# emdgroup/tnmf

Hardware: AMD Instinct MI355X
Metric: MU-iterations/sec (higher is better)
Workload: dtype f32

## Files before the change

### tnmf_amd/csrc/fft.h

```cpp
#pragma once
#include "common.h"

struct FftArgs {
    const void *src0, *src1, *src2;
    void *dst0, *dst1;
    long ps_src, ps_dst;
    int planes, rows, cols;
    int ld_src, ld_dst;
    int KX, KXP;
    int yoff, xoff;
    int N, M, C, Hy;
    int n0, ngroups, nper;
    int mgroups, mper;
    int clamp0;
    double reg;
};

enum FftOp {
    kFftRowsFwd = 0,
    kFftRowsInv,
    kFftRowsInv2,
    kFftRowsMu,
    kFftColsFwd,
    kFftColsInv,
    kFftContractR,
    kFftGradH,
    kFftGradW,
};

typedef int (*fft_run_fn)(int op, int dtype, const FftArgs *a, hipStream_t s);
#define TNMF_FFT_DECL(L) int fft_run_##L(int op, int dtype, const FftArgs *a, hipStream_t s)
TNMF_FFT_DECL(32);
TNMF_FFT_DECL(48);
TNMF_FFT_DECL(64);
TNMF_FFT_DECL(96);
TNMF_FFT_DECL(144);
TNMF_FFT_DECL(192);
TNMF_FFT_DECL(270);
TNMF_FFT_DECL(288);
TNMF_FFT_DECL(384);
TNMF_FFT_DECL(540);
TNMF_FFT_DECL(576);
#undef TNMF_FFT_DECL

bool mixed_has_reconstruct(const Geo &g, int dtype);
bool mixed_has_grad_W(const Geo &g, int dtype);
int mixed_reconstruct(const Geo &g, const void *Tsp, const void *WT, void *OT, int KX, int KXP, hipStream_t s);
int mixed_grad_W(const Geo &g, const void *Tsp, const void *VT, const void *RT, void *Gn, void *Gp, int KX, int KXP,
                 int ngroups, int nper, hipStream_t s);

#ifndef TNMF_MIX_W3_WAVES
#define TNMF_MIX_W3_WAVES 3
#endif
constexpr int kMixW3Atoms = 16, kMixW3Waves = TNMF_MIX_W3_WAVES, kMixW3MaxAy = 12;
constexpr long kMixW3MinBytes = 24L << 20;
constexpr int mix_w3_waves(int Ay) {
    const int w = Ay >= 8 ? 3 : (Ay >= 4 ? 4 : (Ay >= 2 ? 5 : 7));
    return kMixW3Waves < 3 ? kMixW3Waves : w;
}
bool mixed_grad_W3_takes(const Geo &g, int KXP);

int spectral_contract_R(const Geo &g, int dtype, const void *SH, const void *SW, void *SR, int Ly, int KX, int KXP,
                        hipStream_t s);
int spectral_grad_W(const Geo &g, int dtype, const void *SH, const void *SV, const void *SR, void *Gn, void *Gp, int Ly,
                    int KX, int KXP, int ngroups, int nper, hipStream_t s);

bool fft_has(const Geo &g, int dtype);
void fft_invalidate(tnmf_hip_ctx *ctx);
void fft_invalidate_H(tnmf_hip_ctx *ctx, const Geo &g, int dtype, const void *H);
void fft_bind(tnmf_hip_ctx *ctx, const Geo &g, int dtype, const void *H, const void *V);
void fft_unbind(tnmf_hip_ctx *ctx);
void fft_invalidate_W(tnmf_hip_ctx *ctx);
void fft_release(tnmf_hip_ctx *ctx);
int fft_reserve(tnmf_hip_ctx *ctx, const Geo &g, int dtype, bool with_window);

int fft_reconstruct(tnmf_hip_ctx *ctx, const Geo &g, int dtype, const void *W, const void *H, void *R, bool nonneg,
                    hipStream_t s);
int fft_grad_H(tnmf_hip_ctx *ctx, const Geo &g, int dtype, const void *V, const void *R, const void *W, void *neg,
               void *pos, hipStream_t s);
int fft_update_H(tnmf_hip_ctx *ctx, const Geo &g, int dtype, const void *V, const void *R, const void *W, void *H,
                 double reg, hipStream_t s);
int fft_grad_W(tnmf_hip_ctx *ctx, const Geo &g, int dtype, const void *V, const void *R, const void *H, void *neg,
               void *pos, bool nonneg, hipStream_t s);
```

### tnmf_amd/csrc/fft_mixed.hip

```cpp
#include "fft.h"

namespace {

typedef float f2v __attribute__((ext_vector_type(2)));
template <typename T>
struct cplx_of;
template <>
struct cplx_of<float> {
    using type = f2v;
};
template <typename T>
using cplx = typename cplx_of<T>::type;

__device__ __forceinline__ void cfma(f2v &acc, f2v a, f2v b) {
    asm("v_pk_fma_f32 %0, %1, %2, %0 op_sel:[0,0,0] op_sel_hi:[0,1,1]" : "+v"(acc) : "v"(a), "v"(b));
    asm("v_pk_fma_f32 %0, %1, %2, %0 op_sel:[1,1,0] op_sel_hi:[1,0,1] neg_lo:[0,1,0]" : "+v"(acc) : "v"(a), "v"(b));
}
__device__ __forceinline__ void cfmac(f2v &acc, f2v a, f2v b) {
    asm("v_pk_fma_f32 %0, %1, %2, %0 op_sel:[0,0,0] op_sel_hi:[0,1,1] neg_hi:[0,1,0]" : "+v"(acc) : "v"(a), "v"(b));
    asm("v_pk_fma_f32 %0, %1, %2, %0 op_sel:[1,1,0] op_sel_hi:[1,0,1]" : "+v"(acc) : "v"(a), "v"(b));
}
__device__ __forceinline__ void pfma_lo(f2v &acc, f2v x, f2v b) {
    asm("v_pk_fma_f32 %0, %1, %2, %0 op_sel:[0,0,0] op_sel_hi:[1,0,1]" : "+v"(acc) : "v"(x), "v"(b));
}
__device__ __forceinline__ void pfma_hi(f2v &acc, f2v x, f2v b) {
    asm("v_pk_fma_f32 %0, %1, %2, %0 op_sel:[0,1,0] op_sel_hi:[1,1,1]" : "+v"(acc) : "v"(x), "v"(b));
}

#define CHECK(rc_expr)                  \
    do {                                \
        const int _rc = (rc_expr);      \
        if (_rc != TNMF_OK) return _rc; \
    } while (0)

constexpr int kMixCols = 16;

template <typename T, int AY, int CG, int S, int STRIPS>
__global__ __launch_bounds__(kMixCols *STRIPS, 2) void k_mix_reconstruct(const cplx<T> *Tsp, const cplx<T> *WT,
                                                                      cplx<T> *OT, int M, int C, int Hy, int Dy, int KX,
                                                                      int KXP) {
    const int col = threadIdx.x & (kMixCols - 1), strip = threadIdx.x / kMixCols;
    const int kx = blockIdx.x * kMixCols + col, kxc = min(kx, KX - 1);
    const int y0 = (blockIdx.y * STRIPS + strip) * S, n = blockIdx.z;
    cplx<T> acc[CG][S];
#pragma unroll
    for (int c = 0; c < CG; ++c)
#pragma unroll
        for (int y = 0; y < S; ++y) acc[c][y] = {0, 0};
    static_assert(sizeof(cplx<T>) == 8, "float spectra");
    typedef unsigned u32x2v __attribute__((ext_vector_type(2)));
    auto ld = [](const __amdgpu_buffer_rsrc_t &rs, int lane_off, int row_off) {
        const u32x2v w2 = __builtin_amdgcn_raw_buffer_load_b64(rs, lane_off, row_off, 0);
        const unsigned re = w2[0], im = w2[1];
        return cplx<T>{__builtin_bit_cast(float, re), __builtin_bit_cast(float, im)};
    };
    const int rowb = KXP * 8;
    const long tplane = (long)Hy * KXP, wplane = (long)AY * KXP;
    const int lane_t = (y0 * KXP + kxc) * 8, lane_w = kxc * 8;
    const __amdgpu_buffer_rsrc_t wrs =
        __builtin_amdgcn_make_buffer_rsrc((void *)WT, 0, (int)((long)M * C * wplane * 8), 0x00020000);
    auto plane = [&](int m) {
        return __builtin_amdgcn_make_buffer_rsrc((void *)(Tsp + ((long)n * M + m) * tplane), 0, (int)(tplane * 8),
                                                 0x00020000);
    };
    cplx<T> t[S + AY - 1], tn[S + AY - 1];
    {
        const __amdgpu_buffer_rsrc_t rs = plane(0);
#pragma unroll
        for (int r = 0; r < S + AY - 1; ++r) t[r] = ld(rs, lane_t, r * rowb);
    }
    if constexpr (CG == 1) {
        constexpr int MC = 8, NT = kMixCols * STRIPS, ROWS = MC * AY, PIECES = ROWS * (kMixCols / 2);
        constexpr int NPP = (PIECES + NT - 1) / NT;
        typedef float f4v __attribute__((ext_vector_type(4)));
        __shared__ __align__(16) cplx<T> wl[2][ROWS * kMixCols];
        const cplx<T> *wsrc = WT + blockIdx.x * kMixCols;
        const int wrows = M * AY;
        f4v pre[NPP];
        auto wfetch = [&](int chunk) {
#pragma unroll
            for (int k = 0; k < NPP; ++k) {
                const int p = threadIdx.x + k * NT, row = min(chunk * ROWS + (p >> 3), wrows - 1);
                pre[k] = *reinterpret_cast<const f4v *>(wsrc + (long)row * KXP + 2 * (p & 7));
            }
        };
        auto wpark = [&](int buf) {
#pragma unroll
            for (int k = 0; k < NPP; ++k) {
                const int p = threadIdx.x + k * NT;
                if (p < PIECES) *reinterpret_cast<f4v *>(&wl[buf][(p >> 3) * kMixCols + 2 * (p & 7)]) = pre[k];
            }
        };
        wfetch(0);
        wpark(0);
        __syncthreads();
#pragma unroll 1
        for (int m0 = 0, ch = 0; m0 < M; m0 += MC, ++ch) {
            const int buf = ch & 1;
            const bool more = m0 + MC < M;
            if (more) wfetch(ch + 1);
#pragma unroll 1
            for (int mi = 0; mi < MC; ++mi) {
                const int m = m0 + mi;
                if (m >= M) break;
                cplx<T> w[AY];
#pragma unroll
                for (int a = 0; a < AY; ++a) w[a] = wl[buf][(mi * AY + (AY - 1 - a)) * kMixCols + col];
                {
                    const __amdgpu_buffer_rsrc_t rs = plane(min(m + 1, M - 1));
#pragma unroll
                    for (int r = 0; r < S + AY - 1; ++r) tn[r] = ld(rs, lane_t, r * rowb);
                }
#pragma unroll
                for (int a = 0; a < AY; ++a)
#pragma unroll
                    for (int y = 0; y < S; ++y) cfma(acc[0][y], t[y + a], w[a]);
#pragma unroll
                for (int r = 0; r < S + AY - 1; ++r) t[r] = tn[r];
            }
            if (more) wpark(buf ^ 1);
            __syncthreads();
        }
    } else {
#pragma unroll 1
    for (int m = 0; m < M; ++m) {
        cplx<T> w[CG][AY];
#pragma unroll
        for (int c = 0; c < CG; ++c) {
            const int wbase = ((m * C + min(c, C - 1)) * AY) * rowb;
#pragma unroll
            for (int a = 0; a < AY; ++a) w[c][a] = ld(wrs, lane_w, wbase + (AY - 1 - a) * rowb);
        }
        {
            const __amdgpu_buffer_rsrc_t rs = plane(min(m + 1, M - 1));
#pragma unroll
            for (int r = 0; r < S + AY - 1; ++r) tn[r] = ld(rs, lane_t, r * rowb);
        }
#pragma unroll
        for (int c = 0; c < CG; ++c)
#pragma unroll
            for (int a = 0; a < AY; ++a)
#pragma unroll
                for (int y = 0; y < S; ++y) cfma(acc[c][y], t[y + a], w[c][a]);
#pragma unroll
        for (int r = 0; r < S + AY - 1; ++r) t[r] = tn[r];
    }
    }
    if (kx >= KX) return;
#pragma unroll
    for (int c = 0; c < CG; ++c) {
        if (c >= C) break;
#pragma unroll
        for (int y = 0; y < S; ++y)
            if (y0 + y < Dy) OT[((long)n * C + c) * ((long)Dy * KXP) + (long)(y0 + y) * KXP + kx] = acc[c][y];
    }
}

template <typename T, int CG, int SAMPLES>
__global__ __launch_bounds__(kMixCols *SAMPLES) void k_mix_reconstruct_1d(const cplx<T> *Tsp, const cplx<T> *WT,
                                                                        cplx<T> *OT, int N, int M, int C, int KX,
                                                                        int KXP) {
    const int col = threadIdx.x & (kMixCols - 1), sub = threadIdx.x / kMixCols;
    const int kx = blockIdx.x * kMixCols + col, kxc = min(kx, KX - 1);
    const int n = blockIdx.y * SAMPLES + sub, nc = min(n, N - 1);
    cplx<T> acc[CG];
#pragma unroll
    for (int c = 0; c < CG; ++c) acc[c] = {0, 0};
    const cplx<T> *tp = Tsp + (long)nc * M * KXP + kxc;
    int m = 0;
    for (; m + 4 <= M; m += 4) {
        cplx<T> t[4];
#pragma unroll
        for (int q = 0; q < 4; ++q) t[q] = tp[(long)(m + q) * KXP];
#pragma unroll
        for (int q = 0; q < 4; ++q)
#pragma unroll
            for (int c = 0; c < CG; ++c) cfma(acc[c], t[q], WT[((long)(m + q) * C + min(c, C - 1)) * KXP + kxc]);
    }
    for (; m < M; ++m) {
        const cplx<T> t = tp[(long)m * KXP];
#pragma unroll
        for (int c = 0; c < CG; ++c) cfma(acc[c], t, WT[((long)m * C + min(c, C - 1)) * KXP + kxc]);
    }
    if (kx >= KX || n >= N) return;
#pragma unroll
    for (int c = 0; c < CG; ++c) {
        if (c >= C) break;
        OT[((long)n * C + c) * KXP + kx] = acc[c];
    }
}

template <typename T, int AY>
int launch_mix_reconstruct(const void *Tsp, const void *WT, void *OT, const Geo &g, int KX, int KXP, hipStream_t s) {
    const unsigned tiles = (unsigned)cdiv(KX, kMixCols);
    if constexpr (AY == 1) {
        if (g.Dy == 1) {
            constexpr int SAMPLES = 16;
            hipLaunchKernelGGL((k_mix_reconstruct_1d<T, 3, SAMPLES>), dim3(tiles, (unsigned)cdiv(g.N, SAMPLES)),
                               dim3(kMixCols * SAMPLES), 0, s, (const cplx<T> *)Tsp, (const cplx<T> *)WT, (cplx<T> *)OT,
                               g.N, g.M, g.C, KX, KXP);
            TNMF_LAUNCH_CHECK();
            return TNMF_OK;
        }
    }
    if (g.C == 1) {
        constexpr int S = 16, STRIPS = 8;
        hipLaunchKernelGGL((k_mix_reconstruct<T, AY, 1, S, STRIPS>),
                           dim3(tiles, (unsigned)cdiv(g.Dy, S * STRIPS), (unsigned)g.N), dim3(kMixCols * STRIPS), 0, s,
                           (const cplx<T> *)Tsp, (const cplx<T> *)WT, (cplx<T> *)OT, g.M, g.C, g.Hy, g.Dy, KX, KXP);
    } else {
        constexpr int S = 8, STRIPS = 8;
        hipLaunchKernelGGL((k_mix_reconstruct<T, AY, 3, S, STRIPS>),
                           dim3(tiles, (unsigned)cdiv(g.Dy, S * STRIPS), (unsigned)g.N), dim3(kMixCols * STRIPS), 0, s,
                           (const cplx<T> *)Tsp, (const cplx<T> *)WT, (cplx<T> *)OT, g.M, g.C, g.Hy, g.Dy, KX, KXP);
    }
    TNMF_LAUNCH_CHECK();
    return TNMF_OK;
}

template <typename T, int AY, int CG, int GROUPS>
__global__ __launch_bounds__(kMixCols *GROUPS, 2) void k_mix_grad_W(const cplx<T> *Tsp, const cplx<T> *VT,
                                                                 const cplx<T> *RT, cplx<T> *Gn, cplx<T> *Gp, int N,
                                                                 int M, int C, int Hy, int Dy, int KX, int KXP,
                                                                 int nper) {
    const int col = threadIdx.x & (kMixCols - 1), sub = threadIdx.x / kMixCols;
    const int kx = blockIdx.y * kMixCols + col, kxc = min(kx, KX - 1);
    const int m = blockIdx.x, grp = blockIdx.z * GROUPS + sub;
    cplx<T> an[CG][AY], ap[CG][AY];
#pragma unroll
    for (int c = 0; c < CG; ++c)
#pragma unroll
        for (int a = 0; a < AY; ++a) {
            an[c][a] = {0, 0};
            ap[c][a] = {0, 0};
        }
    const int nbeg = grp * nper, nend = min(N, nbeg + nper);
    const long tplane = (long)Hy * KXP, vplane = (long)Dy * KXP;
    static_assert(CG == 1, "one channel per thread");
#pragma unroll 1
    for (int n = nbeg; n < nend; ++n) {
        const cplx<T> *tp = Tsp + ((long)n * M + m) * tplane;
        const cplx<T> *vp = VT + (long)n * C * vplane, *rp = RT + (long)n * C * vplane;
        cplx<T> t[2 * AY - 1], v[AY], r[AY], tn[AY], vn[AY], rn[AY];
#pragma unroll
        for (int i = 0; i < 2 * AY - 1; ++i) t[i] = tp[(unsigned)(min(i, Hy - 1) * KXP + kxc)];
#pragma unroll
        for (int j = 0; j < AY; ++j) {
            const unsigned o = (unsigned)(min(j, Dy - 1) * KXP + kxc);
            v[j] = vp[o];
            r[j] = rp[o];
        }
#pragma unroll 1
        for (int yb = 0; yb < Dy; yb += AY) {
#pragma unroll
            for (int i = 0; i < AY; ++i) tn[i] = tp[(unsigned)(min(yb + 2 * AY - 1 + i, Hy - 1) * KXP + kxc)];
#pragma unroll
            for (int j = 0; j < AY; ++j) {
                const unsigned o = (unsigned)(min(yb + AY + j, Dy - 1) * KXP + kxc);
                vn[j] = vp[o];
                rn[j] = rp[o];
            }
#pragma unroll
            for (int j = 0; j < AY; ++j) {
                if (yb + j >= Dy) {
                    v[j] = {0, 0};
                    r[j] = {0, 0};
                }
#pragma unroll
                for (int a = 0; a < AY; ++a) {
                    cfmac(an[0][a], t[j + a], v[j]);
                    cfmac(ap[0][a], t[j + a], r[j]);
                }
            }
#pragma unroll
            for (int i = 0; i < AY - 1; ++i) t[i] = t[i + AY];
#pragma unroll
            for (int i = 0; i < AY; ++i) t[AY - 1 + i] = tn[i];
#pragma unroll
            for (int j = 0; j < AY; ++j) {
                v[j] = vn[j];
                r[j] = rn[j];
            }
        }
    }
    if (kx >= KX) return;
    const long gplane = (long)AY * KXP, gsize = (long)M * C * gplane;
#pragma unroll
    for (int c = 0; c < CG; ++c) {
        if (c >= C) break;
#pragma unroll
        for (int a = 0; a < AY; ++a) {
            const long o = (long)grp * gsize + ((long)m * C + c) * gplane + (long)a * KXP + kx;
            Gn[o] = an[c][a];
            Gp[o] = ap[c][a];
        }
    }
}

template <typename T, int AY, int GROUPS>
__global__ __launch_bounds__(kMixCols *GROUPS, 2) void k_mix_grad_W2(const cplx<T> *Tsp, const cplx<T> *VT,
                                                                  const cplx<T> *RT, cplx<T> *Gn, cplx<T> *Gp, int N,
                                                                  int M, int Hy, int Dy, int KX, int KXP, int nper,
                                                                  int gx, int gy, int gz) {
    constexpr int MA = 2, VS = 8, RS = (AY + 4 + VS - 1) / VS * VS, P = VS - 1;
    const int col = threadIdx.x & (kMixCols - 1), sub = threadIdx.x / kMixCols;
    int lin = blockIdx.x;
    {
        const int total = gx * gy * gz, whole = total / 8 * 8;
        if (lin < whole) lin = (lin & 7) * (whole / 8) + (lin >> 3);
    }
    const int bx = lin % gx, by = (lin / gx) % gy, bz = lin / (gx * gy);
    const int kx = by * kMixCols + col, kxc = min(kx, KX - 1);
    const int m0 = bx * MA, grp = bz * GROUPS + sub;
    const int m1 = min(m0 + 1, M - 1);
    cplx<T> an[MA][AY], ap[MA][AY];
#pragma unroll
    for (int q = 0; q < MA; ++q)
#pragma unroll
        for (int a = 0; a < AY; ++a) {
            an[q][a] = {0, 0};
            ap[q][a] = {0, 0};
        }
    static_assert(sizeof(cplx<T>) == 8, "float spectra");
    typedef unsigned u32x2v __attribute__((ext_vector_type(2)));
    const long tplane = (long)Hy * KXP, vplane = (long)Dy * KXP;
    const int nbeg0 = bz * GROUPS * nper, nbeg = nbeg0 + sub * nper;
    const int lane_t = (int)(((long)sub * nper * M * tplane + kxc) * 8);
    const int lane_v = (int)(((long)sub * nper * vplane + kxc) * 8);
    const int rowb = KXP * 8;
    auto ld = [](const __amdgpu_buffer_rsrc_t &rs, int lane_off, int row_off) {
        const u32x2v w = __builtin_amdgcn_raw_buffer_load_b64(rs, lane_off, row_off, 0);
        const unsigned re = w[0], im = w[1];
        return cplx<T>{__builtin_bit_cast(float, re), __builtin_bit_cast(float, im)};
    };
#pragma unroll 1
    for (int nr = 0; nr < nper; ++nr) {
        if (nbeg0 + nr >= N) break;
        if (nbeg + nr >= N) continue;
        const cplx<T> *tb = Tsp + ((long)(nbeg0 + nr) * M + m0) * tplane;
        const __amdgpu_buffer_rsrc_t t0 = __builtin_amdgcn_make_buffer_rsrc((void *)tb, 0, 0x7fffffff, 0x00020000);
        const __amdgpu_buffer_rsrc_t t1 =
            __builtin_amdgcn_make_buffer_rsrc((void *)(tb + (long)(m1 - m0) * tplane), 0, 0x7fffffff, 0x00020000);
        const __amdgpu_buffer_rsrc_t vb =
            __builtin_amdgcn_make_buffer_rsrc((void *)(VT + (long)(nbeg0 + nr) * vplane), 0, 0x7fffffff, 0x00020000);
        const __amdgpu_buffer_rsrc_t rb =
            __builtin_amdgcn_make_buffer_rsrc((void *)(RT + (long)(nbeg0 + nr) * vplane), 0, 0x7fffffff, 0x00020000);
        cplx<T> t[MA][RS], v[VS], r[VS];
#pragma unroll
        for (int i = 0; i < RS - 1; ++i) {
            const int o = min(i, Hy - 1) * rowb;
            t[0][i] = ld(t0, lane_t, o);
            t[1][i] = ld(t1, lane_t, o);
        }
#pragma unroll
        for (int i = 0; i < P; ++i) {
            const int o = min(i, Dy - 1) * rowb;
            v[i] = ld(vb, lane_v, o);
            r[i] = ld(rb, lane_v, o);
        }
#pragma unroll 1
        for (int yb = 0; yb < Dy; yb += RS) {
#pragma unroll
            for (int i = 0; i < RS; ++i) {
                const int y = yb + i;
                if (y >= Dy) break;
                {
                    const int o = min(y + RS - 1, Hy - 1) * rowb;
                    t[0][(i + RS - 1) % RS] = ld(t0, lane_t, o);
                    t[1][(i + RS - 1) % RS] = ld(t1, lane_t, o);
                    const int ov = min(y + P, Dy - 1) * rowb;
                    v[(i + P) % VS] = ld(vb, lane_v, ov);
                    r[(i + P) % VS] = ld(rb, lane_v, ov);
                }
                const cplx<T> vy = v[i % VS], ry = r[i % VS];
#pragma unroll
                for (int a = 0; a < AY; ++a) {
                    cfmac(an[0][a], t[0][(i + a) % RS], vy);
                    cfmac(ap[0][a], t[0][(i + a) % RS], ry);
                    cfmac(an[1][a], t[1][(i + a) % RS], vy);
                    cfmac(ap[1][a], t[1][(i + a) % RS], ry);
                }
            }
        }
    }
    if (kx >= KX) return;
    const long gplane = (long)AY * KXP, gsize = (long)M * gplane;
#pragma unroll
    for (int q = 0; q < MA; ++q) {
        if (m0 + q >= M) break;
#pragma unroll
        for (int a = 0; a < AY; ++a) {
            const long o = (long)grp * gsize + (long)(m0 + q) * gplane + (long)a * KXP + kx;
            Gn[o] = an[q][a];
            Gp[o] = ap[q][a];
        }
    }
}

#if defined(__HIP_DEVICE_COMPILE__)
#define TNMF_MIX_NO_DS_PAIRING __attribute__((target("no-load-store-opt")))
#else
#define TNMF_MIX_NO_DS_PAIRING
#endif
template <typename T, int AY>
__global__ __launch_bounds__(kMixCols *kMixW3Atoms, kMixW3Waves) TNMF_MIX_NO_DS_PAIRING void k_mix_grad_W3(
    const cplx<T> *Tsp, const cplx<T> *VT, const cplx<T> *RT, cplx<T> *Gn, cplx<T> *Gp, int N, int M, int Hy, int Dy,
    int KX, int KXP, int nper, int gx, int gy, int gz) {
    constexpr int NA = kMixW3Atoms, RS = 16, CH = RS, NT = kMixCols * NA;
    static_assert(AY + 4 <= RS && sizeof(cplx<T>) == 8 && NT == 2 * CH * (kMixCols / 2), "ring depth, float spectra");
    const int col = threadIdx.x & (kMixCols - 1), slot = threadIdx.x / kMixCols;
    int lin = blockIdx.x;
    {
        const int total = gx * gy * gz, whole = total / 8 * 8;
        if (lin < whole) lin = (lin & 7) * (whole / 8) + (lin >> 3);
    }
    const int bx = lin % gx, by = (lin / gx) % gy, grp = lin / (gx * gy);
    const int kx = by * kMixCols + col, kxc = min(kx, KX - 1);
    const int m = bx * NA + slot, mc = min(m, M - 1);
    f2v a1[AY], a2[AY], a3[AY];
#pragma unroll
    for (int a = 0; a < AY; ++a) a1[a] = a2[a] = a3[a] = {0, 0};
    typedef unsigned u32x2v __attribute__((ext_vector_type(2)));
    typedef float f4v __attribute__((ext_vector_type(4)));
    const long tplane = (long)Hy * KXP, vplane = (long)Dy * KXP;
    const int nbeg = grp * nper, nend = min(N, nbeg + nper);
    const int lane_t = (int)(((long)(mc - bx * NA) * tplane + kxc) * 8);
    const int rowb = KXP * 8;
    auto ld = [](const __amdgpu_buffer_rsrc_t &rs, int lane_off, int row_off) {
        const u32x2v w = __builtin_amdgcn_raw_buffer_load_b64(rs, lane_off, row_off, 0);
        const unsigned re = w[0], im = w[1];
        return cplx<T>{__builtin_bit_cast(float, re), __builtin_bit_cast(float, im)};
    };
    __shared__ __align__(16) f2v xl[2][3][CH * kMixCols];
    const int prow = threadIdx.x / kMixCols, ppair = (threadIdx.x >> 1) & (kMixCols / 2 - 1), pstream = threadIdx.x & 1;
    const cplx<T> *xsrc = (pstream ? RT : VT) + by * kMixCols + 2 * ppair;
    f4v pre;
    auto xfetch = [&](int n, int chunk) {
        pre = *reinterpret_cast<const f4v *>(xsrc + (long)n * vplane + (long)min(chunk * CH + prow, Dy - 1) * KXP);
    };
    auto xpark = [&](int buf) {
        auto swap1 = [](float v) {
            return __builtin_bit_cast(float,
                                      __builtin_amdgcn_update_dpp(0, __builtin_bit_cast(int, v), 0xB1, 0xf, 0xf, false));
        };
        const float oc = swap1(pstream ? pre[0] : pre[2]), od = swap1(pstream ? pre[1] : pre[3]);
        const float cv = pstream ? oc : pre[0], dv = pstream ? od : pre[1];
        const float cr = pstream ? pre[2] : oc, dr = pstream ? pre[3] : od;
        const int e = prow * kMixCols + 2 * ppair + pstream;
        xl[buf][0][e] = f2v{cv, cr};
        xl[buf][1][e] = f2v{cv + dv, cr + dr};
        xl[buf][2][e] = f2v{cv - dv, cr - dr};
    };
    xfetch(min(nbeg, N - 1), 0);
    xpark(0);
    __syncthreads();
    int buf = 0;
#pragma unroll 1
    for (int n = nbeg; n < nend; ++n) {
        const __amdgpu_buffer_rsrc_t t0 = __builtin_amdgcn_make_buffer_rsrc(
            (void *)(Tsp + ((long)n * M + bx * NA) * tplane), 0, 0x7fffffff, 0x00020000);
        cplx<T> t[RS];
        f2v sp[RS / 2];
#pragma unroll
        for (int i = 0; i < RS - 1; ++i) t[i] = ld(t0, lane_t, min(i, Hy - 1) * rowb);
#pragma unroll
        for (int i = 0; i < AY - 1; ++i) sp[i / 2][i & 1] = t[i][0] + t[i][1];
#pragma unroll 1
        for (int yb = 0; yb < Dy; yb += CH) {
            {
                const bool last = yb + CH >= Dy;
                xfetch(last ? min(n + 1, nend - 1) : n, last ? 0 : yb / CH + 1);
            }
            const f2v *x1 = &xl[buf][0][col], *x2 = &xl[buf][1][col], *x3 = &xl[buf][2][col];
#pragma unroll
            for (int i = 0; i < RS; ++i) {
                const int y = yb + i;
                if (y >= Dy) break;
                t[(i + RS - 1) % RS] = ld(t0, lane_t, min(y + RS - 1, Hy - 1) * rowb);
                {
                    const int j = (i + AY - 1) % RS;
                    sp[j / 2][j & 1] = t[j][0] + t[j][1];
                }
                const f2v c = x1[i * kMixCols], cpd = x2[i * kMixCols], cmd = x3[i * kMixCols];
#pragma unroll
                for (int a = 0; a < AY; ++a) {
                    const int j = (i + a) % RS;
                    if (j & 1)
                        pfma_hi(a1[a], c, sp[j / 2]);
                    else
                        pfma_lo(a1[a], c, sp[j / 2]);
                    pfma_lo(a2[a], cpd, t[j]);
                    pfma_hi(a3[a], cmd, t[j]);
                }
            }
            xpark(buf ^ 1);
            __syncthreads();
            buf ^= 1;
        }
    }
    if (kx >= KX || m >= M) return;
    const long gplane = (long)AY * KXP, gsize = (long)M * gplane;
#pragma unroll
    for (int a = 0; a < AY; ++a) {
        const long o = (long)grp * gsize + (long)m * gplane + (long)a * KXP + kx;
        Gn[o] = cplx<T>{a1[a][0] - a3[a][0], a1[a][0] - a2[a][0]};
        Gp[o] = cplx<T>{a1[a][1] - a3[a][1], a1[a][1] - a2[a][1]};
    }
}

template <typename T, int CG, int GROUPS>
__global__ __launch_bounds__(kMixCols *GROUPS) void k_mix_grad_W_1d(const cplx<T> *Tsp, const cplx<T> *VT, const cplx<T> *RT,
                                                                  cplx<T> *Gn, cplx<T> *Gp, int N, int M, int C, int KX,
                                                                  int KXP, int nper) {
    const int col = threadIdx.x & (kMixCols - 1), sub = threadIdx.x / kMixCols;
    const int kx = blockIdx.y * kMixCols + col, kxc = min(kx, KX - 1);
    const int m = blockIdx.x, grp = blockIdx.z * GROUPS + sub;
    cplx<T> an[CG], ap[CG];
#pragma unroll
    for (int c = 0; c < CG; ++c) {
        an[c] = {0, 0};
        ap[c] = {0, 0};
    }
    const int nbeg = grp * nper, nend = min(N, nbeg + nper);
    for (int n = nbeg; n < nend; ++n) {
        const cplx<T> t = Tsp[((long)n * M + m) * KXP + kxc];
#pragma unroll
        for (int c = 0; c < CG; ++c) {
            const long o = ((long)n * C + min(c, C - 1)) * KXP + kxc;
            cfmac(an[c], t, VT[o]);
            cfmac(ap[c], t, RT[o]);
        }
    }
    if (kx >= KX) return;
    const long gsize = (long)M * C * KXP;
#pragma unroll
    for (int c = 0; c < CG; ++c) {
        if (c >= C) break;
        const long o = (long)grp * gsize + ((long)m * C + c) * KXP + kx;
        Gn[o] = an[c];
        Gp[o] = ap[c];
    }
}

template <typename T, int AY>
int launch_mix_grad_W(const void *Tsp, const void *VT, const void *RT, void *Gn, void *Gp, const Geo &g, int KX,
                      int KXP, int ngroups, int nper, hipStream_t s) {
    constexpr int GROUPS = 4;
    if constexpr (AY == 1) {
        if (g.Dy == 1) {
            const dim3 grid((unsigned)g.M, (unsigned)cdiv(KX, kMixCols), (unsigned)cdiv(ngroups, GROUPS));
            hipLaunchKernelGGL((k_mix_grad_W_1d<T, 4, GROUPS>), grid, dim3(kMixCols * GROUPS), 0, s, (const cplx<T> *)Tsp,
                               (const cplx<T> *)VT, (const cplx<T> *)RT, (cplx<T> *)Gn, (cplx<T> *)Gp, g.N, g.M, g.C, KX,
                               KXP, nper);
            TNMF_LAUNCH_CHECK();
            return TNMF_OK;
        }
    }
    if constexpr (AY <= kMixW3MaxAy) {
        if (mixed_grad_W3_takes(g, KXP)) {
            const int gx = cdiv(g.M, kMixW3Atoms), gy = cdiv(KX, kMixCols), gz = ngroups;
            hipLaunchKernelGGL((k_mix_grad_W3<T, AY>), dim3((unsigned)(gx * gy * gz)), dim3(kMixCols * kMixW3Atoms),
                               kMixW3Waves == 2 ? 48u << 10 : 0u, s,
                               (const cplx<T> *)Tsp, (const cplx<T> *)VT, (const cplx<T> *)RT, (cplx<T> *)Gn,
                               (cplx<T> *)Gp, g.N, g.M, g.Hy, g.Dy, KX, KXP, nper, gx, gy, gz);
            TNMF_LAUNCH_CHECK();
            return TNMF_OK;
        }
    }
    if constexpr (AY <= 12) {
        const long span = ((long)(GROUPS - 1) * nper * g.M + 2) * g.Hy * KXP * 8;
        if (g.C == 1 && span < (1L << 31)) {
            const int gx = cdiv(g.M, 2), gy = cdiv(KX, kMixCols), gz = cdiv(ngroups, GROUPS);
            hipLaunchKernelGGL((k_mix_grad_W2<T, AY, GROUPS>), dim3((unsigned)(gx * gy * gz)), dim3(kMixCols * GROUPS), 0, s,
                               (const cplx<T> *)Tsp, (const cplx<T> *)VT, (const cplx<T> *)RT, (cplx<T> *)Gn,
                               (cplx<T> *)Gp, g.N, g.M, g.Hy, g.Dy, KX, KXP, nper, gx, gy, gz);
            TNMF_LAUNCH_CHECK();
            return TNMF_OK;
        }
    }
    const dim3 grid((unsigned)g.M, (unsigned)cdiv(KX, kMixCols), (unsigned)cdiv(ngroups, GROUPS));
    hipLaunchKernelGGL((k_mix_grad_W<T, AY, 1, GROUPS>), grid, dim3(kMixCols * GROUPS), 0, s, (const cplx<T> *)Tsp,
                       (const cplx<T> *)VT, (const cplx<T> *)RT, (cplx<T> *)Gn, (cplx<T> *)Gp, g.N, g.M, g.C, g.Hy, g.Dy,
                       KX, KXP, nper);
    TNMF_LAUNCH_CHECK();
    return TNMF_OK;
}

#define MIX_SWITCH(FN, ...)                                   \
    switch (g.Ay) {                                           \
        case 1: return FN<float, 1>(__VA_ARGS__);             \
        case 2: return FN<float, 2>(__VA_ARGS__);             \
        case 3: return FN<float, 3>(__VA_ARGS__);             \
        case 4: return FN<float, 4>(__VA_ARGS__);             \
        case 5: return FN<float, 5>(__VA_ARGS__);             \
        case 6: return FN<float, 6>(__VA_ARGS__);             \
        case 7: return FN<float, 7>(__VA_ARGS__);             \
        case 8: return FN<float, 8>(__VA_ARGS__);             \
        case 9: return FN<float, 9>(__VA_ARGS__);             \
        case 10: return FN<float, 10>(__VA_ARGS__);           \
        case 11: return FN<float, 11>(__VA_ARGS__);           \
        case 12: return FN<float, 12>(__VA_ARGS__);           \
        case 13: return FN<float, 13>(__VA_ARGS__);           \
        case 14: return FN<float, 14>(__VA_ARGS__);           \
        case 15: return FN<float, 15>(__VA_ARGS__);           \
        case 16: return FN<float, 16>(__VA_ARGS__);           \
        default: return TNMF_E_UNSUPPORTED;                   \
    }

}

bool mixed_has_reconstruct(const Geo &g, int dtype) {
    return dtype == 0 && g.Ay <= 16 && (g.C == 1 || (g.Dy == 1 && g.Ay == 1 && g.C <= 3));
}
bool mixed_has_grad_W(const Geo &g, int dtype) {
    return dtype == 0 && g.Ay <= 16 && (g.C == 1 || (g.Dy == 1 && g.Ay == 1 && g.C <= 4));
}

bool mixed_grad_W3_takes(const Geo &g, int KXP) {
#ifdef TNMF_MIX_NO_W3
    return false;
#endif
    const long span = (long)kMixW3Atoms * g.Hy * KXP * 8;
    const long spectra = (long)g.N * g.M * g.Hy * KXP * 8;
    return g.C == 1 && g.Ay <= kMixW3MaxAy && !(g.Dy == 1 && g.Ay == 1) && span < (1L << 31) && spectra >= kMixW3MinBytes;
}

int mixed_reconstruct(const Geo &g, const void *Tsp, const void *WT, void *OT, int KX, int KXP, hipStream_t s) {
    MIX_SWITCH(launch_mix_reconstruct, Tsp, WT, OT, g, KX, KXP, s);
}

int mixed_grad_W(const Geo &g, const void *Tsp, const void *VT, const void *RT, void *Gn, void *Gp, int KX, int KXP,
                 int ngroups, int nper, hipStream_t s) {
    MIX_SWITCH(launch_mix_grad_W, Tsp, VT, RT, Gn, Gp, g, KX, KXP, ngroups, nper, s);
}
```

Measured before the change: 217.0.

## Add LDS-staged mixed reconstruct kernel with buffer-load prefetch for large spectra

Adds a new reconstruct kernel that stages each atom's spectral rows and W taps into shared memory, using 128-bit buffer loads prefetched one atom ahead. Strips then read overlapping rows from LDS instead of re-reading global memory. It is chosen for C==1, Ay<=12 and spectra of at least 24 MiB. Dynamic shared memory is padded so that about three workgroups fit per CU. The cost is an extra barrier per atom and higher LDS use, which may limit occupancy.

```diff
diff --git a/tnmf_amd/csrc/fft.h b/tnmf_amd/csrc/fft.h
--- a/tnmf_amd/csrc/fft.h
+++ b/tnmf_amd/csrc/fft.h
@@ -60,6 +60,31 @@
 }
 bool mixed_grad_W3_takes(const Geo &g, int KXP);
 
+#ifndef TNMF_MIX_RSH_STRIPS
+#define TNMF_MIX_RSH_STRIPS 16
+#endif
+#ifndef TNMF_MIX_RSH_TILES
+#define TNMF_MIX_RSH_TILES 1
+#endif
+#ifndef TNMF_MIX_RSH_PER_CU
+#define TNMF_MIX_RSH_PER_CU 3
+#endif
+#ifndef TNMF_MIX_RSH_FENCE
+#define TNMF_MIX_RSH_FENCE 0
+#endif
+#ifndef TNMF_MIX_RSH_AUX
+#define TNMF_MIX_RSH_AUX 2
+#endif
+constexpr int kMixRShStrips = TNMF_MIX_RSH_STRIPS, kMixRShTiles = TNMF_MIX_RSH_TILES, kMixRShPerCU = TNMF_MIX_RSH_PER_CU;
+constexpr int kMixRShFence = TNMF_MIX_RSH_FENCE, kMixRShAux = TNMF_MIX_RSH_AUX;
+constexpr int kMixRShWaves = kMixRShPerCU * kMixRShStrips / 16, kMixRShMaxAy = 12;
+constexpr long kMixRShMinBytes = 24L << 20;
+constexpr unsigned mix_rsh_lds_bytes(int Ay) {
+    return kMixRShTiles * (((16 * kMixRShStrips + Ay - 1) * 17 + 1) / 2 * 2 + Ay * 16) * 8u;
+}
+constexpr int mix_rsh_waves(int Ay) { return kMixRShWaves; }
+bool mixed_reconstruct_sh_takes(const Geo &g, int KXP);
+
 int spectral_contract_R(const Geo &g, int dtype, const void *SH, const void *SW, void *SR, int Ly, int KX, int KXP,
                         hipStream_t s);
 int spectral_grad_W(const Geo &g, int dtype, const void *SH, const void *SV, const void *SR, void *Gn, void *Gp, int Ly,
diff --git a/tnmf_amd/csrc/fft_mixed.hip b/tnmf_amd/csrc/fft_mixed.hip
--- a/tnmf_amd/csrc/fft_mixed.hip
+++ b/tnmf_amd/csrc/fft_mixed.hip
@@ -156,6 +156,92 @@
     }
 }
 
+#if defined(__HIP_DEVICE_COMPILE__)
+#define TNMF_MIX_NO_DS_PAIRING __attribute__((target("no-load-store-opt")))
+#else
+#define TNMF_MIX_NO_DS_PAIRING
+#endif
+
+template <typename T, int AY, int STRIPS, int TILES>
+__global__ __launch_bounds__(kMixCols *STRIPS, kMixRShWaves) TNMF_MIX_NO_DS_PAIRING void k_mix_reconstruct_sh(
+    const cplx<T> *Tsp, const cplx<T> *WT, cplx<T> *OT, int M, int Hy, int Dy, int KX, int KXP) {
+    constexpr int S = 16, NT = kMixCols * STRIPS, ROWS = S * STRIPS + AY - 1, PITCH = kMixCols + 1;
+    constexpr int SEG = kMixCols / 2;
+    constexpr int PIECES = ROWS * SEG, NPP = (PIECES + NT - 1) / NT, WPIECES = AY * SEG;
+    constexpr int TROWS = (ROWS * PITCH + 1) / 2 * 2, TILE = TROWS + AY * kMixCols;
+    static_assert(sizeof(cplx<T>) == 8 && WPIECES <= NT && (TILES == 1 || TILES == 2), "float spectra, one W piece per thread");
+    static_assert(STRIPS != kMixRShStrips || TILES != kMixRShTiles || TILES * TILE * 8 == mix_rsh_lds_bytes(AY), "fft.h");
+    typedef unsigned u32x4v __attribute__((ext_vector_type(4)));
+    typedef float f4v __attribute__((ext_vector_type(4)));
+    __shared__ __align__(16) cplx<T> tile[TILES][TILE];
+    const int col = threadIdx.x & (kMixCols - 1), strip = threadIdx.x / kMixCols;
+    const int kx = blockIdx.x * kMixCols + col, colc = min(kx, KX - 1) - blockIdx.x * kMixCols;
+    const int yb = blockIdx.y * (S * STRIPS), y0 = yb + strip * S, n = blockIdx.z;
+    cplx<T> acc[S];
+#pragma unroll
+    for (int y = 0; y < S; ++y) acc[y] = {0, 0};
+    const long tplane = (long)Hy * KXP, wplane = (long)AY * KXP;
+    auto trow = [](int k) { return min((int)(threadIdx.x + k * NT) / SEG, ROWS - 1); };
+    const int pcol = (blockIdx.x * kMixCols + 2 * (threadIdx.x & (SEG - 1))) * 8;
+    int toff[NPP];
+#pragma unroll
+    for (int k = 0; k < NPP; ++k) toff[k] = min(yb + trow(k), Hy - 1) * (KXP * 8) + pcol;
+    const int wrow = min((int)threadIdx.x / SEG, AY - 1), woff = wrow * (KXP * 8) + pcol;
+    f4v pre[NPP], wpre;
+    auto fetch = [&](int m) {
+        const __amdgpu_buffer_rsrc_t rs = __builtin_amdgcn_make_buffer_rsrc(
+            (void *)(Tsp + ((long)n * M + m) * tplane), 0, (int)(tplane * 8), 0x00020000);
+        const __amdgpu_buffer_rsrc_t ws =
+            __builtin_amdgcn_make_buffer_rsrc((void *)(WT + m * wplane), 0, (int)(wplane * 8), 0x00020000);
+#pragma unroll
+        for (int k = 0; k < NPP; ++k)
+            pre[k] = __builtin_bit_cast(f4v, (u32x4v)__builtin_amdgcn_raw_buffer_load_b128(rs, toff[k], 0, kMixRShAux));
+        wpre = __builtin_bit_cast(f4v, (u32x4v)__builtin_amdgcn_raw_buffer_load_b128(ws, woff, 0, 0));
+    };
+    auto park = [&](int buf) {
+        cplx<T> *tl = tile[buf];
+#pragma unroll
+        for (int k = 0; k < NPP; ++k) {
+            const int e = trow(k) * PITCH + 2 * (threadIdx.x & (SEG - 1));
+            tl[e] = cplx<T>{pre[k][0], pre[k][1]};
+            tl[e + 1] = cplx<T>{pre[k][2], pre[k][3]};
+        }
+        *reinterpret_cast<f4v *>(&tl[TROWS + wrow * kMixCols + 2 * (threadIdx.x & (SEG - 1))]) = wpre;
+    };
+    fetch(0);
+    park(0);
+    __syncthreads();
+    const int mine = strip * S * PITCH + colc;
+#pragma unroll 1
+    for (int m = 0; m < M; ++m) {
+        const int buf = TILES == 2 ? (m & 1) : 0;
+        fetch(min(m + 1, M - 1));
+        const cplx<T> *tl = &tile[buf][mine], *wl = &tile[buf][TROWS + colc];
+        cplx<T> w[AY], t[S + AY - 1];
+#pragma unroll
+        for (int r = 0; r < S; ++r) t[r] = tl[r * PITCH];
+        w[0] = wl[(AY - 1) * kMixCols];
+#pragma unroll
+        for (int a = 1; a < AY; ++a) {
+            t[S - 1 + a] = tl[(S - 1 + a) * PITCH];
+            w[a] = wl[(AY - 1 - a) * kMixCols];
+            if (a == kMixRShFence) __builtin_amdgcn_sched_barrier(0);
+        }
+        if (kMixRShFence >= AY) __builtin_amdgcn_sched_barrier(0);
+#pragma unroll
+        for (int a = 0; a < AY; ++a)
+#pragma unroll
+            for (int y = 0; y < S; ++y) cfma(acc[y], t[y + a], w[a]);
+        if (TILES == 1) __syncthreads();
+        park(TILES == 2 ? buf ^ 1 : 0);
+        __syncthreads();
+    }
+    if (kx >= KX) return;
+#pragma unroll
+    for (int y = 0; y < S; ++y)
+        if (y0 + y < Dy) OT[(long)n * ((long)Dy * KXP) + (long)(y0 + y) * KXP + kx] = acc[y];
+}
+
 template <typename T, int CG, int SAMPLES>
 __global__ __launch_bounds__(kMixCols *SAMPLES) void k_mix_reconstruct_1d(const cplx<T> *Tsp, const cplx<T> *WT,
                                                                         cplx<T> *OT, int N, int M, int C, int KX,
@@ -199,6 +285,19 @@
             hipLaunchKernelGGL((k_mix_reconstruct_1d<T, 3, SAMPLES>), dim3(tiles, (unsigned)cdiv(g.N, SAMPLES)),
                                dim3(kMixCols * SAMPLES), 0, s, (const cplx<T> *)Tsp, (const cplx<T> *)WT, (cplx<T> *)OT,
                                g.N, g.M, g.C, KX, KXP);
+            TNMF_LAUNCH_CHECK();
+            return TNMF_OK;
+        }
+    }
+    if constexpr (AY <= kMixRShMaxAy) {
+        if (mixed_reconstruct_sh_takes(g, KXP)) {
+            constexpr unsigned tiles_lds = mix_rsh_lds_bytes(AY), hold = (160u << 10) / (kMixRShPerCU + 1) + 1;
+            static_assert(tiles_lds * kMixRShPerCU <= 160u << 10, "the tiles of kMixRShPerCU workgroups fit a CU");
+            hipLaunchKernelGGL((k_mix_reconstruct_sh<T, AY, kMixRShStrips, kMixRShTiles>),
+                               dim3(tiles, (unsigned)cdiv(g.Dy, 16 * kMixRShStrips), (unsigned)g.N),
+                               dim3(kMixCols * kMixRShStrips), tiles_lds < hold ? hold - tiles_lds : 0u, s,
+                               (const cplx<T> *)Tsp, (const cplx<T> *)WT,
+                               (cplx<T> *)OT, g.M, g.Hy, g.Dy, KX, KXP);
             TNMF_LAUNCH_CHECK();
             return TNMF_OK;
         }
@@ -397,11 +496,6 @@
     }
 }
 
-#if defined(__HIP_DEVICE_COMPILE__)
-#define TNMF_MIX_NO_DS_PAIRING __attribute__((target("no-load-store-opt")))
-#else
-#define TNMF_MIX_NO_DS_PAIRING
-#endif
 template <typename T, int AY>
 __global__ __launch_bounds__(kMixCols *kMixW3Atoms, kMixW3Waves) TNMF_MIX_NO_DS_PAIRING void k_mix_grad_W3(
     const cplx<T> *Tsp, const cplx<T> *VT, const cplx<T> *RT, cplx<T> *Gn, cplx<T> *Gp, int N, int M, int Hy, int Dy,
@@ -625,6 +719,15 @@
     return g.C == 1 && g.Ay <= kMixW3MaxAy && !(g.Dy == 1 && g.Ay == 1) && span < (1L << 31) && spectra >= kMixW3MinBytes;
 }
 
+bool mixed_reconstruct_sh_takes(const Geo &g, int KXP) {
+#ifdef TNMF_MIX_NO_RSH
+    return false;
+#endif
+    const long plane = (long)g.Hy * KXP * 8;
+    const long spectra = (long)g.N * g.M * g.Hy * KXP * 8;
+    return g.C == 1 && g.Ay <= kMixRShMaxAy && !(g.Dy == 1 && g.Ay == 1) && plane < (1L << 31) && spectra >= kMixRShMinBytes;
+}
+
 int mixed_reconstruct(const Geo &g, const void *Tsp, const void *WT, void *OT, int KX, int KXP, hipStream_t s) {
     MIX_SWITCH(launch_mix_reconstruct, Tsp, WT, OT, g, KX, KXP, s);
 }
```

Result: faster. 224.3 (median of 6 runs) (+3.4%).
